# evolbioinfo/pastml

Measured on AMD Instinct MI355X. Metric: ACR nodes*states*chars/sec (full marginal pass: P(t) + bottom-up + top-down + posteriors), higher is better.
Workload: dtype f64; 1 GPU; BASELINE config 4 shard: balanced tree, 1048576 tips (2097151 nodes), k=64 states, F81, 32 characters per GPU (32 in total), marginal (BU+TD+posteriors); tips=1048576, nodes=2097151, states=64, chars_per_gpu=32, chars_total=32, substitution_model=F81, collective=local

## Files before the change

### pastml_amd/csrc/pml_api.hip

```cpp
#define PML_PLAIN_KERNELS
#include "pml_launch.h"
#include "pml_kernels_counts.h"
#include "pml_kernels_eigen_gemm.h"
#include "pml_comm.h"
#include "pml_pij_window.h"

#ifndef PML_BUILD_DIGEST
#define PML_BUILD_DIGEST "unknown"
#endif
static const char kBuildDigest[] = "PML_BUILD_DIGEST=" PML_BUILD_DIGEST;

static thread_local std::string g_last_error;

int pml_fail(int code, const char* fmt, ...) {
    char buf[1024];
    va_list ap;
    va_start(ap, fmt);
    vsnprintf(buf, sizeof(buf), fmt, ap);
    va_end(ap);
    g_last_error = buf;
    return code;
}

template <typename T>
// ... 986 lines not shown
    t.C = ctx->C;
    t.sched_cols = ctx->sched_cols;
    t.n_roots = ctx->n_roots;
    t.n_cherries = ctx->n_cherries;
    t.has_init = ctx->has_init;
    t.fuse = ctx->fuse;
    t.Gf = ctx->cols.Gf;
    t.Gt = ctx->cols.Gt;
    t.bu_wide_lanes = ctx->cols.bu_wide_lanes;
    t.level_lists_sorted = ctx->cols.level_lists_sorted;
    t.single_launch = single_launch_sweeps(ctx);
    t.blocks = block_schedule(ctx);
    t.super = super_sweeps(ctx);
    t.thin = thin_bottom_up(ctx);
    t.deep = deep_top_down(ctx);
    t.narrow_units = (int)ctx->tune.get(T_NARROW_UNITS, 0);
    t.no_td_tail = ctx->tune.on(T_NO_TD_TAIL);
    t.no_eigg_tiers = ctx->tune.on(T_NO_EIGG_TIERS);
    t.no_spin_wait = ctx->tune.on(T_NO_SPIN_WAIT);
    t.waves = PML_WAVES_PER_BLOCK;
    const int ks4 = (ctx->k + 3) / 4;
    t.eig_nb = ks4 % 4 == 0 ? 1 : (ks4 % 2 == 0 ? 2 : 4);
    t.td_chain = t.f81 && t.super && ctx->sup.chain_depth >= 0 && !ctx->tune.on(T_NO_TD_CHAIN) && !ctx->tune.on(T_NO_TD_SUPER_PIPE);
    return t;
}

static PmlSchedules schedules_of(const pml_ctx* ctx) {
    return {&ctx->blocks, &ctx->thin, &ctx->deep, &ctx->sup, &ctx->eig_tiers, &ctx->bt_tiers, &ctx->bu_level_vec_f,
            &ctx->bu_level_vec, &ctx->td_cherry_prefix};
}

static int run_plan(pml_ctx* ctx, const std::vector<PmlLaunch>& whole_plan, bool bottom_up, int is_marginal, bool force_prep) {
    const bool windowed = ctx->pij_window > 0 && ctx->kind == PML_MODEL_EIGEN;
    const int wtab = bottom_up ? 0 : 1;
    const std::vector<PmlWindowStep>* cached = nullptr;
    std::vector<PmlLaunch> cut;
    if (windowed) {
        auto same = [](const PmlLaunch& a, const PmlLaunch& b) {
            return a.op == b.op && a.list == b.list && a.kind == b.kind && a.bracket == b.bracket && a.branch == b.branch &&
                   a.signal == b.signal && a.cherries == b.cherries && a.first == b.first && a.count == b.count && a.arg == b.arg;
        };
        for (const pml_ctx::WindowCut& c : ctx->win_cuts)
            if (c.plan.size() == whole_plan.size() && std::equal(c.plan.begin(), c.plan.end(), whole_plan.begin(), same)) cached = &c.steps;
        if (cached == nullptr) {
            PmlWindowPlan W;
            const std::string bad = pml_plan_pij_window(whole_plan, ctx->forest, ctx->bu_order, ctx->td_parents, ctx->pij_window, W);
// ... 3 lines not shown
            if (ctx->win_cuts.size() >= 16) ctx->win_cuts.clear();
            ctx->win_cuts.push_back(pml_ctx::WindowCut{whole_plan, std::move(W.steps)});
            cached = &ctx->win_cuts.back().steps;
        }
        cut.reserve(cached->size());
        for (const PmlWindowStep& w : *cached) cut.push_back(w.launch);
    }
    static const std::vector<PmlWindowStep> no_steps;
    const std::vector<PmlWindowStep>& steps = windowed ? *cached : no_steps;
    const std::vector<PmlLaunch>& plan = windowed ? cut : whole_plan;
    size_t at = 0;
    const pml_ctx::EigenTiers& E = ctx->eig_tiers;
    const pml_ctx::BacktraceTiers& B = ctx->bt_tiers;
    const int* order = bottom_up ? ctx->d_bu_order : nullptr;
    const int* offsets = bottom_up ? ctx->d_bu_offsets : ctx->d_td_offsets;
    const int gemm_mode = bottom_up ? PML_EIGG_BU : PML_EIGG_TD;
    const int eig_mode = !bottom_up ? PML_EIG_TD : (is_marginal ? PML_EIG_BU_MARG : PML_EIG_BU_JOINT);
    int open = PML_NO_BRACKET;
    long long launches = 0;
    for (const PmlLaunch& r : plan) {
        if (ctx->tune.on(T_DEBUG))
            fprintf(stderr, "pml plan: branch %d op %d list %d kind %d first %d count %d arg %d bracket %d signal %d%s\n", r.branch,
                    r.op, r.list, r.kind, r.first, r.count, r.arg, r.bracket, (int)r.signal,
                    r.op == OP_SUPER && !bottom_up && r.arg > 0 ? " (chained: with the stacked units of depth arg - 1)" : "");
        if (r.bracket != open) {
            if (open != PML_NO_BRACKET) PML_TRY(prof_end(ctx, open, launches));
            if (r.bracket != PML_NO_BRACKET) PML_TRY(prof_begin(ctx));
            open = r.bracket;
            launches = 0;
        }
        ++launches;
        const PmlWindowStep* run = windowed ? &steps[at] : nullptr;
        ++at;
        if (run != nullptr && run->build_count > 0) {
            PML_TRY(launch_pij_wide_list(ctx, ctx->d_pij_window, ctx->pij_window, ctx->d_win_branches[wtab] + run->build_first,
                                         run->build_count));
            ++launches;
        }
        const bool joint = r.kind == EIG_JOINT, gemm = r.kind == EIG_GEMM;
        switch (r.op) {
            case OP_RESET_ERR:
                hipLaunchKernelGGL(reset_err_kernel, dim3((ctx->C + 63) / 64), dim3(64), 0, ctx->stream, ctx->d_err, ctx->C,
                                   r.arg ? ctx->d_tip_rest_count : nullptr);
                HIP_TRY(hipGetLastError());
                break;
            case OP_PREP:
                if (!windowed) PML_TRY(run_prep(ctx, force_prep, true));
// ... 3 lines not shown
                                   tree_of(ctx), cols_of(ctx, true), state_of(ctx), ctx->C, is_marginal ? 1 : 0, ctx->h_loglik,
                                   ctx->h_err);
                HIP_TRY(hipGetLastError());
                break;
            case OP_LEVEL:
                PML_TRY(dispatch_sweep(ctx, (SweepKind)r.kind, r.list, r.first, r.count, r.cherries, bottom_up,
                                       windowed && (r.list == L_BU_PLAIN || r.list == L_TD_PLAIN) ? wtab : -1));
                break;
            case OP_ROOTS:
                PML_TRY(dispatch_sweep(ctx, SW_ROOTS, L_NONE, 0, r.count));
                break;
            case OP_LEVELS: {
                const bool whole = r.list == L_BU_FUSED || r.list == L_TD_FUSED;
                const int do_prep = (bottom_up && r.arg && (ctx->results.pij_stale() || force_prep)) ? 1 : 0;
                PML_TRY(dispatch_small_f81(ctx, bottom_up, r.signal, do_prep, whole ? r.first : 0, r.count,
                                           whole ? nullptr : ctx->d_unit_lists[r.list], whole ? nullptr : ctx->d_list_offsets[r.list] + r.first,
                                           bottom_up ? 0 : r.arg));
                break;
            }
            case OP_BLOCKS:
                PML_TRY(dispatch_blocks_f81(ctx, bottom_up, r.first, r.signal));
                break;
            case OP_SUPER:
                PML_TRY(dispatch_super_f81(ctx, bottom_up, bottom_up ? -1 : r.arg - 1));
                break;
            case OP_STACK:
                PML_TRY(dispatch_stack_f81(ctx, bottom_up, r.first));
                break;
            case OP_EIG_TIPS:
                if (joint) PML_TRY(launch_eigen_joint_tips(ctx));
                else if (gemm) PML_TRY(launch_eigen_gemm(ctx, PML_EIGG_TIPS, ctx->d_tips, 0, ctx->n_tips));
                else PML_TRY(launch_eigen_tips(ctx, is_marginal ? 0 : 1));
                break;
            case OP_EIG_LEVEL: {
                const int* nodes = order ? order + r.first : nullptr;
                const int first = order ? 0 : r.first;
                if (joint) PML_TRY(launch_eigen_joint(ctx, ctx->d_bu_units + r.first, nullptr, 0, r.count));
                else if (gemm) PML_TRY(launch_eigen_gemm(ctx, gemm_mode, nodes, first, r.count));
                else PML_TRY(launch_eigen_fused(ctx, eig_mode, nodes, first, r.count, 0));
                break;
            }
            case OP_EIG_NARROW:
                if (joint) PML_TRY(launch_eigen_joint(ctx, ctx->d_bu_units, offsets, r.first, r.count));
                else if (gemm) PML_TRY(launch_eigen_gemm_narrow(ctx, gemm_mode, order, offsets, r.first, r.count));
                else PML_TRY(launch_eigen_narrow(ctx, eig_mode, order, offsets, r.first, r.count));
                break;
            case OP_EIG_TIER: {
// ... 1507 lines not shown
```

### pastml_amd/csrc/pml_kernels_f81.h

```cpp
#pragma once
#include "pml_device.h"
#include "pml_schedule.h"

typedef unsigned char pml_jt;

struct PmlTree {
    int N;
    int n_roots;
    const int* parent;
    const int* first_child;
    const int* n_children;
    const double* dist;
    const int* post_rank;
    const unsigned char* kind;
};

struct PmlCols {
    int k, ks, W;
    int no_wide_lean;
    const u64* masks;
    const u64* masks_init;
    const double* pi;
    const double* active;
};
// ... 1523 lines not shown
template <int G, int R>
__device__ __forceinline__ void bu_f81_super_issue(const LaneCtx<G, R>& L, const SuperRegs& s, SuperLoads<R>& ld) {
#pragma unroll
    for (int j = 0; j < 2; ++j) {
        const UnitRegs u = super_child<G>(s, j, L.g);
        f81_gather_issue<G, R>(L, u, ld.c[j].cl, ld.c[j].tl);
        ld.c[j].own = L.mask[(unsigned)u.n];
    }
    ld.e = L.E[s.fc + (L.g & 1)];
    ld.own = L.mask[(unsigned)s.n];
}

template <int R>
__device__ __forceinline__ void super_loads_arrived(SuperLoads<R>& ld) {
#pragma unroll
    for (int j = 0; j < 2; ++j)
        asm volatile("" : "+v"(ld.c[j].cl.e), "+v"(ld.c[j].cl.mask), "+v"(ld.c[j].tl.e), "+v"(ld.c[j].tl.s),
                          "+v"(ld.c[j].tl.mask), "+v"(ld.c[j].own));
    asm volatile("" : "+v"(ld.e), "+v"(ld.own));
}

template <int G, int R>
__device__ __forceinline__ bool bu_f81_super_unit(const LaneCtx<G, R>& L, const PmlTree& t, const PmlCols& c,
                                                  const PmlState& st, const SuperRegs& s, SuperLoads<R>& ld) {
    super_loads_arrived<R>(ld);
    const u64 kbits = state_bits(c.k);
    bool ones = c.k == G * R;
#pragma unroll
    for (int j = 0; j < 2; ++j) {
        f81_gather_finish<G, R>(L, ld.c[j].cl, ld.c[j].tl);
        ones = ones && (ld.c[j].own & kbits) == kbits && ld.c[j].cl.mask == kbits;
    }
    const bool full = __all(ones);
    BuResult<R> res[2];
#pragma unroll
    for (int j = 0; j < 2; ++j) {
        const UnitRegs u = super_child<G>(s, j, L.g);
        const bool ok = full ? bu_f81_marg_body<G, R, false, true, true>(L, t, c, st, u, ld.c[j], &res[j], false)
                             : bu_f81_marg_body<G, R, false, false, true>(L, t, c, st, u, ld.c[j], &res[j], false);
        if (!ok) return false;
    }
    BuLoads<R> top;
    top.cl.e = ld.e;
    top.cl.s = (L.g & 1) ? res[1].s : res[0].s;
    top.cl.be = (L.g & 1) ? res[1].e : res[0].e;
    top.cl.mask = kbits;
    top.tl.e = top.tl.s = top.tl.a = 0.0;
    top.tl.mask = 0ull;
    top.own = ld.own;
#pragma unroll
    for (int r = 0; r < R; ++r) {
        top.v0[r] = res[0].v[r];
        top.v1[r] = res[1].v[r];
    }
    return bu_f81_marg_body<G, R, true, false>(L, t, c, st, super_own(s), top);
}

template <int G, int R>
__device__ __forceinline__ void bu_f81_super_seq(const LaneCtx<G, R>& L, const PmlTree& t, const PmlCols& c,
                                                 const PmlState& st, const SuperRegs& s) {
    bu_f81_unit_seq<G, R, false>(L, t, c, st, super_child<G>(s, 0, L.g));
    bu_f81_unit_seq<G, R, false>(L, t, c, st, super_child<G>(s, 1, L.g));
    __threadfence();
    bu_f81_unit_seq<G, R, false>(L, t, c, st, super_own(s));
}

template <int G, int R>
__global__ void __launch_bounds__(PML_BLOCK) __attribute__((amdgpu_waves_per_eu(2, 2)))
bu_f81_super_kernel(PmlTree t, PmlCols c, PmlState st, const PmlUnit* __restrict__ units, int n_level) {
    constexpr int UW = 64 / G;
    const int wave = threadIdx.x >> 6;
    const int sub = (threadIdx.x & 63) / G;
    LaneCtx<G, R> L;
    lane_ctx_init<G, R>(L, t, c, st);
    const int stride = gridDim.x * PML_WAVES_PER_BLOCK * UW;
    int idx = (blockIdx.x * PML_WAVES_PER_BLOCK + wave) * UW + sub;
    int base = idx - sub;
    SuperRegs ua = load_super(units, idx < n_level ? idx : 0);
// ... 950 lines not shown
    int n, fc, g0, g1;
};

__device__ __forceinline__ StackRegs load_stack(const PmlUnit* __restrict__ units, int idx) {
    const int4 h = *reinterpret_cast<const int4*>(units + idx);
    const int4 f = *reinterpret_cast<const int4*>(units[idx].cfc);
    StackRegs s;
    s.n = h.x;
    s.fc = h.y;
    s.g0 = f.x;
    s.g1 = f.y;
    return s;
}

__device__ __forceinline__ UnitRegs stack_child(const StackRegs& s, int j) {
    UnitRegs u;
    u.n = s.fc + j;
    u.fc = j ? s.g1 : s.g0;
    u.packed = PML_PACKED_TWO_STORED;
    u.cfc = u.cfc1 = u.cfc2 = u.cfc3 = 0;
    return u;
}

template <int G, int R>
__device__ __forceinline__ void stack_child_loads(const LaneCtx<G, R>& L, const PmlCols& c, int node, int first,
                                                  BuLoads<R>& ld) {
    const int ch = first + (L.g & 1);
    ld.cl.e = L.E[ch];
    ld.cl.s = L.S[ch];
    ld.cl.be = L.be[ch];
    ld.cl.mask = 0ull;
    ld.tl.e = ld.tl.s = ld.tl.a = 0.0;
    ld.tl.mask = 0ull;
    ld.own = L.mask[(unsigned)node];
    node_load_vec<G, R>(L, c, L.bu, first, ld.v0);
    node_load_vec<G, R>(L, c, L.bu, first + 1, ld.v1);
}

template <int G, int R>
__device__ __forceinline__ bool bu_f81_stack_unit(const LaneCtx<G, R>& L, const PmlTree& t, const PmlCols& c,
                                                  const PmlState& st, const StackRegs& s) {
    BuLoads<R> ld[2];
#pragma unroll
    for (int j = 0; j < 2; ++j) stack_child_loads<G, R>(L, c, s.fc + j, j ? s.g1 : s.g0, ld[j]);
    const double e_top = L.E[s.fc + (L.g & 1)];
    const u64 own = L.mask[(unsigned)s.n];
    BuResult<R> res[2];
#pragma unroll
    for (int j = 0; j < 2; ++j)
        if (!bu_f81_marg_body<G, R, true, false>(L, t, c, st, stack_child(s, j), ld[j], &res[j], false)) return false;
    BuLoads<R> top;
    top.cl.e = e_top;
    top.cl.s = (L.g & 1) ? res[1].s : res[0].s;
    top.cl.be = (L.g & 1) ? res[1].e : res[0].e;
    top.cl.mask = 0ull;
    top.tl.e = top.tl.s = top.tl.a = 0.0;
    top.tl.mask = 0ull;
    top.own = own;
#pragma unroll
    for (int r = 0; r < R; ++r) {
        top.v0[r] = res[0].v[r];
        top.v1[r] = res[1].v[r];
    }
    UnitRegs un;
    un.n = s.n;
    un.fc = s.fc;
    un.packed = PML_PACKED_TWO_STORED;
    un.cfc = un.cfc1 = un.cfc2 = un.cfc3 = 0;
    return bu_f81_marg_body<G, R, true, false>(L, t, c, st, un, top);
}

template <int G, int R>
__global__ void __launch_bounds__(PML_BLOCK) __attribute__((amdgpu_waves_per_eu(2, 2)))
bu_f81_stack_kernel(PmlTree t, PmlCols c, PmlState st, const PmlUnit* __restrict__ units, int n_level) {
    constexpr int UW = 64 / G;
    const int wave = threadIdx.x >> 6;
    const int sub = (threadIdx.x & 63) / G;
    LaneCtx<G, R> L;
    lane_ctx_init<G, R>(L, t, c, st);
    const int stride = gridDim.x * PML_WAVES_PER_BLOCK * UW;
    int idx = (blockIdx.x * PML_WAVES_PER_BLOCK + wave) * UW + sub;
    StackRegs cur = load_stack(units, idx < n_level ? idx : 0);
    for (int base = idx - sub; base < n_level; base += stride) {
        const int nxt_idx = idx + stride;
        const StackRegs nxt = load_stack(units, nxt_idx < n_level ? nxt_idx : 0);
        if (idx < n_level) {
            if (!bu_f81_stack_unit<G, R>(L, t, c, st, cur)) {
                bu_f81_unit_seq<G, R, false>(L, t, c, st, stack_child(cur, 0));
                bu_f81_unit_seq<G, R, false>(L, t, c, st, stack_child(cur, 1));
                __threadfence();
                UnitRegs un = stack_child(cur, 0);
                un.n = cur.n;
                un.fc = cur.fc;
                bu_f81_unit_seq<G, R, false>(L, t, c, st, un);
            }
        }
        cur = nxt;
        idx = nxt_idx;
    }
}

struct TdRowNowhere {
    template <int G, int R>
    __device__ __forceinline__ void operator()(const LaneCtx<G, R>&, const PmlCols&, int, const double (&)[R], double, i64) const {}
};
#define PML_TD_CHAIN_SLOT(G, R) ((G) * (R) + 2)
struct TdRowToLds {
    double* slots;
    template <int G, int R>
    __device__ __forceinline__ void operator()(const LaneCtx<G, R>& L, const PmlCols& c, int jx, const double (&po)[R], double ls,
                                               i64 le) const {
        double* row = slots + jx * PML_TD_CHAIN_SLOT(G, R);
#pragma unroll
        for (int r = 0; r < R; r += 2) {
            double2 t2;
            t2.x = L.st(r) < c.ks ? po[r] : 0.0;
            t2.y = L.st(r) < c.ks ? po[r + 1] : 0.0;
            *reinterpret_cast<double2*>(row + L.st(r)) = t2;
        }
        if (L.g == 0) {
            row[G * R] = ls;
// ... 400 lines not shown
```

### pastml_amd/csrc/pml_launch.h

```cpp
#pragma once
#include "pml_host.h"
#include "pml_time_segments.h"

#define PML_GR_CASES(X)  \
    X(8, 4)              \
    X(1, 1)              \
    X(2, 1)              \
    X(4, 1)              \
    X(8, 1)              \
    X(16, 1)             \
    X(64, 1)             \
    X(32, 2)             \
    X(64, 2)             \
    X(64, 4)


#define PML_F81_CASES(X) \
    X(2, 2)              \
    X(4, 2)              \
    X(1, 1)              \
    X(1, 2)              \
    X(1, 4)              \
    X(2, 4)              \
    X(4, 4)              \
// ... 33 lines not shown

static bool eigen_gemm(const pml_ctx* c) {
    const bool off = c->tune.on(T_NO_EIGEN_GEMM) || c->tune.on(T_NO_MFMA) || c->tune.on(T_NO_EIGEN_FUSED);
    if (off || !c->eig_fused_opt || c->kind != PML_MODEL_EIGEN || c->k < 2) return false;
    if (c->k <= 64) return c->W == 1;
    return c->k <= 128 && c->W == 2 && c->eig_sym_all && c->d_Asym != nullptr;
}


static bool eigen_joint_valu(const pml_ctx* c) {
    const bool off = c->tune.on(T_NO_EIGEN_JOINT_VALU);
    return !off && c->eigj_valu_opt && c->kind == PML_MODEL_EIGEN && c->k >= 2 && c->k <= 64 && c->W == 1 &&
           c->d_AinvT != nullptr;
}


PML_INTERNAL int dispatch_sweep_matrix(pml_ctx* ctx, SweepKind what, const int* level, int n_level, int window = -1);
PML_INTERNAL int dispatch_select(pml_ctx* ctx, int method, int force_joint, const u64* d_lh_mask);
PML_INTERNAL int dispatch_sweep_f81(pml_ctx* ctx, SweepKind what, const PmlUnit* units, int n_level, bool cherries, bool bu_sweep);
PML_INTERNAL int dispatch_sweep_f81_wide(pml_ctx* ctx, SweepKind what, const PmlUnit* units, int n_level, bool cherries, bool bu_sweep);
PML_INTERNAL int dispatch_small_f81(pml_ctx* ctx, bool bottom_up, bool signal, int do_prep, int first_level, int n_levels,
                                    const PmlUnit* units = nullptr, const int* d_offsets = nullptr, int skip_roots = 0);
PML_INTERNAL int dispatch_blocks_f81(pml_ctx* ctx, bool bottom_up, int which, bool signal);
PML_INTERNAL int dispatch_super_f81(pml_ctx* ctx, bool bottom_up, int chain_depth = -1);
PML_INTERNAL int dispatch_stack_f81(pml_ctx* ctx, bool bottom_up, int level);
PML_INTERNAL int launch_eigen_fused(pml_ctx* ctx, int mode, const int* nodes, int first, int n, int tips);
PML_INTERNAL int launch_eigen_narrow(pml_ctx* ctx, int mode, const int* nodes, const int* d_offsets, int first_level, int n_levels);
PML_INTERNAL int launch_eigen_tips(pml_ctx* ctx, int joint);
PML_INTERNAL int launch_pij_mfma(pml_ctx* ctx);
PML_INTERNAL int launch_pij_wide(pml_ctx* ctx);
PML_INTERNAL int launch_pij_wide_list(pml_ctx* ctx, double* window, long long B, const int* d_branches, int count, int col_begin = 0,
                                      int col_end = -1);
PML_INTERNAL int arm_pij_wide_list(pml_ctx* ctx);
PML_INTERNAL int launch_eigen_gemm(pml_ctx* ctx, int mode, const int* nodes, int first, int n);
PML_INTERNAL int launch_eigen_gemm_narrow(pml_ctx* ctx, int mode, const int* nodes, const int* d_offsets, int first_level,
                                          int n_levels, const int* d_blk_start = nullptr, int n_blocks = 1);
PML_INTERNAL int launch_eigen_gemm_wide(pml_ctx* ctx, int mode, const int* nodes, int first, int n);
PML_INTERNAL int launch_eigen_gemm_narrow_wide(pml_ctx* ctx, int mode, const int* nodes, const int* d_offsets, int first_level,
                                               int n_levels, const int* d_blk_start, int n_blocks);
PML_INTERNAL int launch_eigen_joint(pml_ctx* ctx, const PmlUnit* units, const int* d_offsets, int first, int n,
                                    const int* d_blk_start = nullptr, int n_blocks = 1);
PML_INTERNAL int launch_eigen_joint_tips(pml_ctx* ctx);
PML_INTERNAL int launch_pij_valu(pml_ctx* ctx);
PML_INTERNAL int launch_simulate(pml_ctx* ctx, int col, int rep_offset, u64 seed, void* d_states, size_t rs);
PML_INTERNAL int sim_frontier_depth(const pml_ctx* ctx, int n_tiles);
PML_INTERNAL int sim_subtree_lists(pml_ctx* ctx, int D);
static inline bool pij_windowed(const pml_ctx* ctx) {
// ... 94 lines not shown
```

### pastml_amd/csrc/pml_launch_f81_super.hip

```cpp
#include "pml_launch.h"

template <int G, int R, bool LANES, bool PIPE>
static void launch_td_super_f81(pml_ctx* ctx, dim3 grid, const PmlTree& t, const PmlCols& c, const PmlState& st) {
    hipLaunchKernelGGL((td_f81_super_kernel<G, R, LANES, PIPE>), grid, dim3(PML_BLOCK), 0, ctx->stream, t, c, st, ctx->sup.d_units,
                       ctx->sup.n);
}

template <int G, int R>
static void launch_td_chain_f81(pml_ctx* ctx, int a, const PmlTree& t, const PmlCols& c, const PmlState& st) {
    const int tiles = (2 * ctx->sup.n + 4 * (64 / G) - 1) / (4 * (64 / G));
    dim3 grid(grid_for(ctx, tiles, PML_WAVES_PER_BLOCK, ctx->C, true), ctx->C);
    if (!ctx->tune.on(T_NO_TIP_LANES))
        hipLaunchKernelGGL((td_f81_chain_kernel<G, R, true>), grid, dim3(PML_BLOCK), 0, ctx->stream, t, c, st, ctx->sup.d_units,
                           ctx->sup.n, ctx->sup.d_stack_td + a);
    else
        hipLaunchKernelGGL((td_f81_chain_kernel<G, R, false>), grid, dim3(PML_BLOCK), 0, ctx->stream, t, c, st, ctx->sup.d_units,
                           ctx->sup.n, ctx->sup.d_stack_td + a);
}

template <int G, int R>
static void launch_super_f81(pml_ctx* ctx, bool bottom_up, int chain_first) {
    const PmlTree t = tree_of(ctx, true);
    const PmlCols c = cols_of(ctx, bottom_up);
    const PmlState st = state_of(ctx);
    if (chain_first >= 0) return launch_td_chain_f81<G, R>(ctx, chain_first, t, c, st);
    const int upb = PML_WAVES_PER_BLOCK * (64 / G);
    const bool pipe = bottom_up || !ctx->tune.on(T_NO_TD_SUPER_PIPE);
    dim3 grid(grid_for(ctx, bottom_up ? ctx->sup.n : 2 * ctx->sup.n, upb, ctx->C, pipe), ctx->C), block(PML_BLOCK);
    const bool lanes = !ctx->tune.on(T_NO_TIP_LANES);
    if (bottom_up)
        hipLaunchKernelGGL((bu_f81_super_kernel<G, R>), grid, block, 0, ctx->stream, t, c, st, ctx->sup.d_units, ctx->sup.n);
    else if (pipe && lanes)
        launch_td_super_f81<G, R, true, true>(ctx, grid, t, c, st);
    else if (pipe)
        launch_td_super_f81<G, R, false, true>(ctx, grid, t, c, st);
    else if (lanes)
        launch_td_super_f81<G, R, true, false>(ctx, grid, t, c, st);
    else
        launch_td_super_f81<G, R, false, false>(ctx, grid, t, c, st);
}

template <int G, int R>
static void launch_stack_f81(pml_ctx* ctx, bool bottom_up, int a, int n) {
    const PmlTree t = tree_of(ctx, true);
    const PmlCols c = cols_of(ctx, bottom_up);
    const PmlState st = state_of(ctx);
    const int upb = PML_WAVES_PER_BLOCK * (64 / G);
    dim3 grid(grid_for(ctx, bottom_up ? n : 2 * n, upb, ctx->C), ctx->C), block(PML_BLOCK);
    if (bottom_up)
        hipLaunchKernelGGL((bu_f81_stack_kernel<G, R>), grid, block, 0, ctx->stream, t, c, st, ctx->sup.d_stack_bu + a, n);
    else
        hipLaunchKernelGGL((td_f81_stack_kernel<G, R>), grid, block, 0, ctx->stream, t, c, st, ctx->sup.d_stack_td + a, n);
}

int dispatch_super_f81(pml_ctx* ctx, bool bottom_up, int chain_depth) {
    if (ctx->sup.n <= 0) return PML_OK;
    int chain_first = -1;
    if (chain_depth >= 0) {
        const std::vector<int>& off = ctx->sup.stack_td_offsets;
        if (bottom_up || chain_depth != ctx->sup.chain_depth || chain_depth + 1 >= (int)off.size() ||
            (long long)(off[chain_depth + 1] - off[chain_depth]) * 4 != ctx->sup.n)
            return fail(PML_ERR_INVALID, "no chained two-level launch for depth %d", chain_depth);
        chain_first = off[chain_depth];
    }
    const auto [g, r] = ctx->cols.shape(bottom_up);
#define X(G_, R_)                                                \
    if (g == G_ && r == R_) {                                    \
        launch_super_f81<G_, R_>(ctx, bottom_up, chain_first);   \
        HIP_TRY(hipGetLastError());                              \
        return PML_OK;                                           \
    }
    PML_SUPER_CASES(X)
#undef X
    return fail(PML_ERR_UNSUPPORTED, "no two-level F81 kernel for G=%d R=%d", g, r);
}

int dispatch_stack_f81(pml_ctx* ctx, bool bottom_up, int level) {
    const std::vector<int>& off = bottom_up ? ctx->sup.stack_bu_offsets : ctx->sup.stack_td_offsets;
    if (ctx->sup.n_stack == 0 || level + 1 >= (int)off.size()) return PML_OK;
    const int a = off[level], n = off[level + 1] - a;
    if (n <= 0) return PML_OK;
    const auto [g, r] = ctx->cols.shape(bottom_up);
#define X(G_, R_)                                         \
    if (g == G_ && r == R_) {                             \
        launch_stack_f81<G_, R_>(ctx, bottom_up, a, n);   \
        HIP_TRY(hipGetLastError());                       \
// ... 8 lines not shown
```

### pastml_amd/csrc/pml_schedule.cpp

```cpp
#include "pml_schedule.h"
#include "pml_columns.h"

#include <algorithm>
#include <cstdarg>
#include <cstdio>

static std::string message(const char* fmt, ...) __attribute__((format(printf, 1, 2)));
static std::string message(const char* fmt, ...) {
    char buf[1024];
    va_list ap;
    va_start(ap, fmt);
    vsnprintf(buf, sizeof(buf), fmt, ap);
    va_end(ap);
    return buf;
}

std::string pml_check_tree(const PmlTreeArrays& t) {
    const int n_nodes = t.n_nodes, n_roots = t.n_roots, n_bu_levels = t.n_bu_levels, n_td_levels = t.n_td_levels;
    const int *parent = t.parent, *first_child = t.first_child, *n_children = t.n_children, *bu_offsets = t.bu_offsets,
              *bu_order = t.bu_order, *td_offsets = t.td_offsets, *td_parent_offsets = t.td_parent_offsets,
              *td_parents = t.td_parents, *post_rank = t.post_rank;
    if (n_nodes <= 0 || n_roots <= 0 || n_roots > n_nodes) return "bad node/root counts";
    if (!parent || !first_child || !n_children || !t.dist || !bu_offsets || !td_offsets || !td_parent_offsets || !post_rank)
        return "NULL tree array";
// ... 453 lines not shown
        const std::vector<int> depth_of = node_depths(f);
        U.stack_bu_offsets.assign(max_h + 1, 0);
        for (int n : stack_list) ++U.stack_bu_offsets[fh[n]];
        for (int l = 0; l < max_h; ++l) U.stack_bu_offsets[l + 1] += U.stack_bu_offsets[l];
        std::vector<int> by_depth(stack_list);
        std::stable_sort(by_depth.begin(), by_depth.end(), [&](int x, int y) { return depth_of[x] < depth_of[y]; });
        U.stack_td_offsets.assign(n_td_levels + 1, 0);
        for (int n : by_depth) ++U.stack_td_offsets[depth_of[n] + 1];
        for (int l = 0; l < n_td_levels; ++l) U.stack_td_offsets[l + 1] += U.stack_td_offsets[l];
        P.sup.stack_bu = describe(f, stack_list);
        P.sup.stack_td = describe(f, by_depth);
        P.sup.stack_children = describe(f, stack_children);
        U.n_stack = (int)stack_list.size();
        int deepest = n_td_levels - 1;
        while (deepest >= 0 && U.stack_td_offsets[deepest + 1] == U.stack_td_offsets[deepest]) --deepest;
        const int a = U.stack_td_offsets[deepest], cnt = U.stack_td_offsets[deepest + 1] - a;
        bool lined_up = (long long)cnt * 4 == (long long)sup_list.size();
        for (int m = 0; m < cnt && lined_up; ++m) {
            const int n = by_depth[a + m], g0 = fc[fc[n]], g1 = fc[fc[n] + 1];
            lined_up = sup_list[4 * m] == g0 && sup_list[4 * m + 1] == g0 + 1 && sup_list[4 * m + 2] == g1 &&
                       sup_list[4 * m + 3] == g1 + 1;
        }
        if (lined_up) U.chain_depth = deepest;
        if (tune.on(T_DEBUG)) fprintf(stderr, "pastml_hip: %d stacked units, chain depth %d\n", U.n_stack, U.chain_depth);
    }
    if (sup_list.empty() && stack_list.empty()) return;
    std::vector<int> bu_r, td_r;
    U.bu_offsets_r.assign(1, 0);
    for (int l = 0; l < max_h; ++l) {
        for (int q = off[l]; q < off[l + 1]; ++q)
            if (!gone[order[q]]) bu_r.push_back(order[q]);
        U.bu_offsets_r.push_back((int)bu_r.size());
    }
    U.td_offsets_r.assign(1, 0);
    for (int l = 0; l < n_td_levels; ++l) {
        for (int q = f.td_parent_offsets_f[l]; q < f.td_parent_offsets_f[l + 1]; ++q)
            if (!gone[f.tdp[q]]) td_r.push_back(f.tdp[q]);
        U.td_offsets_r.push_back((int)td_r.size());
    }
    for (int n : sup_list) {
        sup_children.push_back(fc[n]);
        sup_children.push_back(fc[n] + 1);
    }
    U.n_child_units = (int)sup_children.size();
    P.sup.child_units = describe(f, sup_children);
    P.sup.bu_units_r = describe(f, bu_r);
    P.sup.td_units_r = describe(f, td_r);
// ... 313 lines not shown
    };
    auto narrow_end = [&](int list, int first_level, int tail) {
        p.bracket = PML_NO_BRACKET;
        if (tail > 0) p.add(OP_LEVELS, list, first_level, tail).signal = t.sched_cols <= 64 && !t.no_spin_wait;
    };
    switch (p.branch) {
        case BU_ONE_LAUNCH: {
            PmlLaunch& r = p.add(OP_LEVELS, L_BU_FUSED, 0, nl);
            r.arg = 1;
            r.signal = t.sched_cols <= 64 && !t.no_spin_wait;
            break;
        }
        case BU_BLOCKS: {
            const PmlBlockSchedule& B = *s.blocks;
            p.add(OP_BLOCKS, L_NONE, 0, B.n_blocks);
            const int n = (int)B.top_bu_offsets.size() - 1;
            const int tail = narrow_levels(t, B.top_bu_offsets, n, false, t.sched_cols);
            p.levels(OP_LEVEL, L_TOP_BU, B.top_bu_offsets, 0, n - tail, true, marg_kind(B.top_bu_vec));
            narrow_end(L_TOP_BU, n - tail, tail);
            break;
        }
        case BU_SUPER: {
            const PmlSuperSchedule& U = *s.sup;
            p.bracket = 4;
            if (U.n > 0) p.add(OP_SUPER, L_NONE, 0, U.n);
            p.bracket = 0;
            const int n = (int)U.bu_offsets_r.size() - 1;
            int tail = narrow_levels(t, U.bu_offsets_r, n, false, t.sched_cols);
            for (int l = n - 1; l >= 0 && U.n_stack > 0; --l)
                if (U.stack_bu_offsets[l + 1] > U.stack_bu_offsets[l]) {
                    tail = std::min(tail, n - 1 - l);
                    break;
                }
            if (tail < 2) tail = 0;
            p.levels(OP_LEVEL, t.level_lists_sorted ? L_REST_BU_SORTED : L_REST_BU, U.bu_offsets_r, 0, n - tail, false,
                     marg_kind(U.bu_level_vec_r), [&](int l) { add_stack(p, U, U.stack_bu_offsets, l); });
            narrow_end(L_REST_BU, n - tail, tail);
            break;
        }
        case BU_THIN: {
            const PmlThinSchedule& H = *s.thin;
            p.levels(OP_LEVEL, fused_list, f.bu_offsets_f, 0, H.floor_level, true, marg_kind(*s.bu_level_vec_f));
            for (size_t q = 0; q < H.tiers.size(); ++q) p.add(OP_BLOCKS, L_NONE, 1 + (int)q, H.tiers[q].n_blocks);
            const int tail = std::min(nl - H.top_level, narrow_levels(t, f.bu_offsets_f, nl, false, t.sched_cols));
            p.levels(OP_LEVEL, fused_list, f.bu_offsets_f, H.top_level, nl - tail, true, marg_kind(*s.bu_level_vec_f));
            narrow_end(L_BU_FUSED, nl - tail, tail);
            break;
        }
        case BU_FUSED: {
            const int tail = narrow_levels(t, f.bu_offsets_f, nl, false, t.sched_cols);
            p.levels(OP_LEVEL, fused_list, f.bu_offsets_f, 0, nl - tail, true, marg_kind(*s.bu_level_vec_f));
            narrow_end(L_BU_FUSED, nl - tail, tail);
            break;
        }
        case BU_FUSED_JOINT:
            p.levels(OP_LEVEL, L_BU_FUSED, f.bu_offsets_f, 0, nl, true,
                     [&](int l) { return (int)((*s.bu_level_vec_f)[l] ? SW_BU_JOINT_FUSED : SW_BU_JOINT_FUSED_NOVEC); });
            break;
        case BU_EIGJ_TIERS:
// ... 129 lines not shown
```

### pastml_amd/csrc/pml_schedule.h

```cpp
#pragma once
#include <cstdlib>
#include <string>
#include <vector>

#define PML_KIND_TIP 0
#define PML_KIND_CHERRY 1
#define PML_KIND_STORED 2

struct __attribute__((aligned(32))) PmlUnit {
    int n, fc, packed, pad;
    int cfc[4];
};

#define PML_PACKED_TWO_STORED ((1 << 11) | (1 << 8) | (3 << 4) | 2)

#define PML_SMALL_BLOCK 512

#define PML_TUNABLES(X)                                                                                              \
    X(GRID_CAP, 0, 0) X(SMALL_MANY_NODES, 0, 0) X(BLOCK_MAX_WORK, 0, 0)    \
    X(NO_MFMA, 1, 0) X(NO_EIGEN_FUSED, 1, 0) X(NO_HKY_FUSED, 1, 0)      \
    X(BLOCK_THREADS, 0, 0) X(EIG_BLOCKS, 0, 0) X(NO_EIGEN_GEMM, 1, 0) X(NO_EIGEN_JOINT_VALU, 1, 0) X(EIGJ_BLOCKS, 0, 0) \
    X(EIGJ_TIP_BLOCKS, 0, 0) X(EIGJ_ONE_TIPS_KERNEL, 1, 0) X(EIGJ_TIER_THIN, 0, 1) X(EIGJ_TIER_DEPTH, 0, 1)            \
    X(NO_EIGJ_TIERS, 1, 1) X(NO_BT_TIERS, 1, 1) X(NO_SHAPE_SORT, 1, 1) X(NO_SUPER, 1, 1) X(SUPER_MIN, 0, 1)            \
    X(STACK_MIN, 0, 1) X(NO_STACK, 1, 1) X(DEBUG, 1, 0) X(BLOCK_NODES, 0, 1) X(BLOCK_MAX_STORED, 0, 1)                 \
    X(BLOCK_HEIGHT_CAP, 0, 1) X(SMALL_MAX_NODES, 0, 1) X(F81_R, 0, 1) X(F81_TD_R, 0, 1) X(NO_GRAPH, 1, 1)              \
    X(NARROW_UNITS, 0, 0) X(NO_EIGG_TIERS, 1, 0) X(NO_SPIN_WAIT, 1, 0)   \
    X(PIJ_STAGE_ROWS, 0, 0) X(PIJ_BLOCKS, 0, 0) X(NO_HEIGHT_ORDER, 1, 1) X(NO_TD_TAIL, 1, 0) X(NO_PIJ_VALU, 1, 0) X(PIJ_VALU, 1, 0) X(NO_PIJ_WIDE, 1, 0) X(NO_EIGJ_PIPE, 1, 0) \
    X(THIN_UNITS, 0, 1) X(THIN_BYTES, 0, 1) X(THIN_BLOCK_NODES, 0, 1) X(NO_THIN, 1, 0) X(NO_THIN_WIDE, 1, 0) X(BU_WIDE, 0, 1) X(SORT_LEVELS, 0, 1) X(NO_WIDE_LEAN, 1, 0) X(SHAPE_ORDER, 0, 1) \
    X(PARS_MAX_COLS, 0, 0) X(PARS_THIN, 0, 0) X(COMPRESS_MAX_COLS, 0, 0) X(COMPRESS_PLAIN_ATOMICS, 1, 0) \
    X(PIJ_WINDOW, 0, 0) X(NO_KEEP_TIP_ROWS, 1, 0) X(NO_TIP_LANES, 1, 0) X(NO_TD_SUPER_PIPE, 1, 0) X(NO_TD_CHAIN, 1, 0)
enum PmlTunable {
#define X(name, flag, tree) T_##name,
    PML_TUNABLES(X)
#undef X
    T_COUNT
};
static const char* const kTunableName[T_COUNT] = {
#define X(name, flag, tree) #name,
    PML_TUNABLES(X)
#undef X
};
static const bool kTunableFlag[T_COUNT] = {
#define X(name, flag, tree) flag != 0,
    PML_TUNABLES(X)
#undef X
};
static const bool kTunableTree[T_COUNT] = {
#define X(name, flag, tree) tree != 0,
    PML_TUNABLES(X)
#undef X
};
struct PmlTune {
    long long val[T_COUNT];
// ... 29 lines not shown
    struct Tier { int first_block, n_blocks; };
    std::vector<Tier> tiers;
    PmlUnit* d_units = nullptr;
    int *d_start = nullptr, *d_levels = nullptr, *d_lv = nullptr;
};
struct PmlDeepSchedule {
    bool ok = false;
    int first_depth = 0, n_blocks = 0;
    PmlUnit* d_units = nullptr;
    int *d_start = nullptr, *d_levels = nullptr, *d_lv = nullptr;
};
struct PmlSuperSchedule {
    bool ok = false;
    int n = 0;
    PmlUnit* d_units = nullptr;
    PmlUnit* d_child_units = nullptr;
    PmlUnit *d_bu_units_r = nullptr, *d_td_units_r = nullptr;
    PmlUnit *d_bu_units_rs = nullptr, *d_td_units_rs = nullptr;
    int n_child_units = 0;
    int n_stack = 0;
    PmlUnit *d_stack_bu = nullptr, *d_stack_td = nullptr, *d_stack_children = nullptr;
    std::vector<int> stack_bu_offsets, stack_td_offsets;
    int chain_depth = -1;
    int *d_bu_offsets_r = nullptr, *d_td_offsets_r = nullptr;
    std::vector<int> bu_offsets_r, td_offsets_r;
    std::vector<char> bu_level_vec_r;
};
struct PmlEigenTiers {
    bool ok = false;
    int first_level = 0;
    int top_level = 0;
    struct Tier { int first_block, n_blocks, depth; };
    std::vector<Tier> tiers;
    PmlUnit* d_units = nullptr;
    int *d_lv = nullptr, *d_start = nullptr;
    int* d_nodes = nullptr;
    int widest = 0;
};
struct PmlBacktraceTiers {
    bool ok = false;
    int first_depth = 0;
    struct Tier { int first_block, n_blocks, depth; };
    std::vector<Tier> tiers;
    int *d_nodes = nullptr, *d_lv = nullptr, *d_start = nullptr;
};

// ... 126 lines not shown
struct PmlSweepOutcome {
    int n_signals = 0;
    bool final_signals = false;
    bool has_params = false;
    bool fused_joint = false;
    void then(const PmlSweepOutcome& next) {
        n_signals += next.n_signals;
        final_signals = next.final_signals;
        has_params = has_params || next.has_params;
        fused_joint = fused_joint || next.fused_joint;
    }
};
struct PmlSweepTraits {
    bool f81, eigen_fused, eigen_gemm, eigen_joint_valu, hky_fused, wide_states;
    int k, W, C, sched_cols, n_roots, n_cherries;
    bool has_init, fuse;
    int Gf, Gt;
    bool bu_wide_lanes, level_lists_sorted;
    bool single_launch, blocks, super, thin, deep;
    int narrow_units;
    bool no_td_tail, no_eigg_tiers, no_spin_wait;
    int waves, eig_nb;
    bool td_chain;
};
struct PmlSchedules {
    const PmlBlockSchedule* blocks;
    const PmlThinSchedule* thin;
    const PmlDeepSchedule* deep;
    const PmlSuperSchedule* sup;
    const PmlEigenTiers* eig;
    const PmlBacktraceTiers* bt;
    const std::vector<char>*bu_level_vec_f, *bu_level_vec;
    const std::vector<int>* td_cherry_prefix;
};

#define PML_PLAN __attribute__((visibility("hidden")))
PML_PLAN std::string pml_check_tree(const PmlTreeArrays& t);
PML_PLAN PmlForest pml_plan_forest(PmlTreeArrays& t, const PmlTune& tune, bool fuse, PmlNumbering& num);
PML_PLAN PmlTreePlan pml_plan_tree(const PmlForest& f, const PmlTreeArrays& t, const PmlTune& tune);
PML_PLAN PmlThinPlan pml_plan_thin_ends(const PmlForest& f, const PmlTune& tune, int thin);
PML_PLAN std::vector<PmlLaunch> pml_plan_bottom_up(const PmlForest& f, const PmlSchedules& s, const PmlSweepTraits& t, bool is_marginal);
PML_PLAN std::vector<PmlLaunch> pml_plan_top_down(const PmlForest& f, const PmlSchedules& s, const PmlSweepTraits& t, bool wants_signal);
PML_PLAN std::vector<PmlLaunch> pml_plan_backtrace(const PmlForest& f, const PmlSchedules& s, const PmlSweepTraits& t, int* head);
PML_PLAN PmlSweepOutcome pml_plan_outcome(const std::vector<PmlLaunch>& plan);
```

Measured before the change: 628.8 billion node*state*char/s.

## Chain bottom-up super units with the first stacked level via LDS in one kernel

Adds a bottom-up chained kernel that processes four super units per stacked unit and passes their partial likelihood vectors and scale scalars through shared memory to the stacked parent, instead of writing them to global memory and launching a separate stack kernel. The scheduler detects when the lowest stacked level lines up exactly with the super list and skips that level's separate stack launch. Loads for the stack step (edge factors, masks) are prefetched while the supers run. This removes a kernel launch and a global round trip of child vectors, but it adds LDS use, fixes 2 waves per block and needs a fallback path from global memory when any lane had to take the sequential route.

```diff
diff --git a/pastml_amd/csrc/pml_api.hip b/pastml_amd/csrc/pml_api.hip
--- a/pastml_amd/csrc/pml_api.hip
+++ b/pastml_amd/csrc/pml_api.hip
@@ -1032,6 +1032,7 @@
     const int ks4 = (ctx->k + 3) / 4;
     t.eig_nb = ks4 % 4 == 0 ? 1 : (ks4 % 2 == 0 ? 2 : 4);
     t.td_chain = t.f81 && t.super && ctx->sup.chain_depth >= 0 && !ctx->tune.on(T_NO_TD_CHAIN) && !ctx->tune.on(T_NO_TD_SUPER_PIPE);
+    t.bu_chain = t.f81 && t.super && ctx->sup.bu_chain_level >= 0 && !ctx->tune.on(T_NO_BU_CHAIN);
     return t;
 }
 
@@ -1081,7 +1082,8 @@
         if (ctx->tune.on(T_DEBUG))
             fprintf(stderr, "pml plan: branch %d op %d list %d kind %d first %d count %d arg %d bracket %d signal %d%s\n", r.branch,
                     r.op, r.list, r.kind, r.first, r.count, r.arg, r.bracket, (int)r.signal,
-                    r.op == OP_SUPER && !bottom_up && r.arg > 0 ? " (chained: with the stacked units of depth arg - 1)" : "");
+                    r.op != OP_SUPER || r.arg <= 0 ? "" : bottom_up ? " (chained: with the stacked units of level arg - 1)"
+                                                                    : " (chained: with the stacked units of depth arg - 1)");
         if (r.bracket != open) {
             if (open != PML_NO_BRACKET) PML_TRY(prof_end(ctx, open, launches));
             if (r.bracket != PML_NO_BRACKET) PML_TRY(prof_begin(ctx));
@@ -1131,7 +1133,7 @@
                 PML_TRY(dispatch_blocks_f81(ctx, bottom_up, r.first, r.signal));
                 break;
             case OP_SUPER:
-                PML_TRY(dispatch_super_f81(ctx, bottom_up, bottom_up ? -1 : r.arg - 1));
+                PML_TRY(dispatch_super_f81(ctx, bottom_up, r.arg - 1));
                 break;
             case OP_STACK:
                 PML_TRY(dispatch_stack_f81(ctx, bottom_up, r.first));
diff --git a/pastml_amd/csrc/pml_kernels_f81.h b/pastml_amd/csrc/pml_kernels_f81.h
--- a/pastml_amd/csrc/pml_kernels_f81.h
+++ b/pastml_amd/csrc/pml_kernels_f81.h
@@ -1569,7 +1569,8 @@
 
 template <int G, int R>
 __device__ __forceinline__ bool bu_f81_super_unit(const LaneCtx<G, R>& L, const PmlTree& t, const PmlCols& c,
-                                                  const PmlState& st, const SuperRegs& s, SuperLoads<R>& ld) {
+                                                  const PmlState& st, const SuperRegs& s, SuperLoads<R>& ld,
+                                                  BuResult<R>* keep = nullptr) {
     super_loads_arrived<R>(ld);
     const u64 kbits = state_bits(c.k);
     bool ones = c.k == G * R;
@@ -1600,7 +1601,7 @@
         top.v0[r] = res[0].v[r];
         top.v1[r] = res[1].v[r];
     }
-    return bu_f81_marg_body<G, R, true, false>(L, t, c, st, super_own(s), top);
+    return bu_f81_marg_body<G, R, true, false>(L, t, c, st, super_own(s), top, keep, true);
 }
 
 template <int G, int R>
@@ -2597,29 +2598,111 @@
     return u;
 }
 
-template <int G, int R>
+struct BuKidsFromMemory {
+    template <int G, int R>
+    __device__ __forceinline__ void scalars(const LaneCtx<G, R>& L, int, int ch, double& s, i64& be) const {
+        s = L.S[ch];
+        be = L.be[ch];
+    }
+    template <int G, int R>
+    __device__ __forceinline__ void vectors(const LaneCtx<G, R>& L, const PmlCols& c, int, int first, double (&v0)[R],
+                                            double (&v1)[R]) const {
+        node_load_vec<G, R>(L, c, L.bu, first, v0);
+        node_load_vec<G, R>(L, c, L.bu, first + 1, v1);
+    }
+};
+#define PML_BU_CHAIN_SLOT(G, R) ((G) * (R) + 2)
+struct BuKidsFromLds {
+    const double* slots;
+    template <int G, int R>
+    __device__ __forceinline__ void scalars(const LaneCtx<G, R>& L, int j, int, double& s, i64& be) const {
+        const double* row = slots + (2 * j + (L.g & 1)) * PML_BU_CHAIN_SLOT(G, R);
+        s = row[G * R];
+        be = *reinterpret_cast<const i64*>(row + G * R + 1);
+    }
+    template <int G, int R>
+    __device__ __forceinline__ void vectors(const LaneCtx<G, R>& L, const PmlCols&, int j, int, double (&v0)[R],
+                                            double (&v1)[R]) const {
+        const double* row = slots + 2 * j * PML_BU_CHAIN_SLOT(G, R);
+#pragma unroll
+        for (int r = 0; r < R; r += 2) {
+            const double2 a = *reinterpret_cast<const double2*>(row + L.st(r));
+            const double2 b = *reinterpret_cast<const double2*>(row + PML_BU_CHAIN_SLOT(G, R) + L.st(r));
+            v0[r] = a.x;
+            v0[r + 1] = a.y;
+            v1[r] = b.x;
+            v1[r + 1] = b.y;
+        }
+    }
+};
+struct BuKidsOfChain {
+    const double* slots;
+    bool from_memory;
+    template <int G, int R>
+    __device__ __forceinline__ void scalars(const LaneCtx<G, R>& L, int j, int ch, double& s, i64& be) const {
+        if (from_memory) BuKidsFromMemory().scalars<G, R>(L, j, ch, s, be);
+        else BuKidsFromLds{slots}.scalars<G, R>(L, j, ch, s, be);
+    }
+    template <int G, int R>
+    __device__ __forceinline__ void vectors(const LaneCtx<G, R>& L, const PmlCols& c, int j, int first, double (&v0)[R],
+                                            double (&v1)[R]) const {
+        if (from_memory) BuKidsFromMemory().vectors<G, R>(L, c, j, first, v0, v1);
+        else BuKidsFromLds{slots}.vectors<G, R>(L, c, j, first, v0, v1);
+    }
+};
+template <int G, int R>
+__device__ __forceinline__ void bu_chain_slot_store(const LaneCtx<G, R>& L, const PmlCols& c, double* row, const BuResult<R>& res) {
+#pragma unroll
+    for (int r = 0; r < R; r += 2) {
+        double2 t2;
+        t2.x = L.st(r) < c.ks ? res.v[r] : 0.0;
+        t2.y = L.st(r) < c.ks ? res.v[r + 1] : 0.0;
+        *reinterpret_cast<double2*>(row + L.st(r)) = t2;
+    }
+    if (L.g == 0) {
+        row[G * R] = res.s;
+        *reinterpret_cast<i64*>(row + G * R + 1) = res.e;
+    }
+}
+
+struct StackAhead {
+    double e[2], e_top;
+    u64 own[2], own_top;
+};
+template <int G, int R>
+__device__ __forceinline__ void stack_ahead_issue(const LaneCtx<G, R>& L, const StackRegs& s, StackAhead& a) {
+#pragma unroll
+    for (int j = 0; j < 2; ++j) {
+        a.e[j] = L.E[(j ? s.g1 : s.g0) + (L.g & 1)];
+        a.own[j] = L.mask[(unsigned)(s.fc + j)];
+    }
+    a.e_top = L.E[s.fc + (L.g & 1)];
+    a.own_top = L.mask[(unsigned)s.n];
+}
+
+template <int G, int R, class Kids = BuKidsFromMemory>
 __device__ __forceinline__ void stack_child_loads(const LaneCtx<G, R>& L, const PmlCols& c, int node, int first,
-                                                  BuLoads<R>& ld) {
+                                                  BuLoads<R>& ld, const Kids& kids = Kids(), int j = 0,
+                                                  const StackAhead* ahead = nullptr) {
     const int ch = first + (L.g & 1);
-    ld.cl.e = L.E[ch];
-    ld.cl.s = L.S[ch];
-    ld.cl.be = L.be[ch];
+    ld.cl.e = ahead != nullptr ? ahead->e[j] : L.E[ch];
+    kids.template scalars<G, R>(L, j, ch, ld.cl.s, ld.cl.be);
     ld.cl.mask = 0ull;
     ld.tl.e = ld.tl.s = ld.tl.a = 0.0;
     ld.tl.mask = 0ull;
-    ld.own = L.mask[(unsigned)node];
-    node_load_vec<G, R>(L, c, L.bu, first, ld.v0);
-    node_load_vec<G, R>(L, c, L.bu, first + 1, ld.v1);
-}
-
-template <int G, int R>
+    ld.own = ahead != nullptr ? ahead->own[j] : L.mask[(unsigned)node];
+    kids.template vectors<G, R>(L, c, j, first, ld.v0, ld.v1);
+}
+
+template <int G, int R, class Kids = BuKidsFromMemory>
 __device__ __forceinline__ bool bu_f81_stack_unit(const LaneCtx<G, R>& L, const PmlTree& t, const PmlCols& c,
-                                                  const PmlState& st, const StackRegs& s) {
+                                                  const PmlState& st, const StackRegs& s, const Kids& kids = Kids(),
+                                                  const StackAhead* ahead = nullptr) {
     BuLoads<R> ld[2];
 #pragma unroll
-    for (int j = 0; j < 2; ++j) stack_child_loads<G, R>(L, c, s.fc + j, j ? s.g1 : s.g0, ld[j]);
-    const double e_top = L.E[s.fc + (L.g & 1)];
-    const u64 own = L.mask[(unsigned)s.n];
+    for (int j = 0; j < 2; ++j) stack_child_loads<G, R>(L, c, s.fc + j, j ? s.g1 : s.g0, ld[j], kids, j, ahead);
+    const double e_top = ahead != nullptr ? ahead->e_top : L.E[s.fc + (L.g & 1)];
+    const u64 own = ahead != nullptr ? ahead->own_top : L.mask[(unsigned)s.n];
     BuResult<R> res[2];
 #pragma unroll
     for (int j = 0; j < 2; ++j)
@@ -2643,6 +2726,18 @@
     un.packed = PML_PACKED_TWO_STORED;
     un.cfc = un.cfc1 = un.cfc2 = un.cfc3 = 0;
     return bu_f81_marg_body<G, R, true, false>(L, t, c, st, un, top);
+}
+
+template <int G, int R>
+__device__ __forceinline__ void bu_f81_stack_seq(const LaneCtx<G, R>& L, const PmlTree& t, const PmlCols& c,
+                                                 const PmlState& st, const StackRegs& s) {
+    bu_f81_unit_seq<G, R, false>(L, t, c, st, stack_child(s, 0));
+    bu_f81_unit_seq<G, R, false>(L, t, c, st, stack_child(s, 1));
+    __threadfence();
+    UnitRegs un = stack_child(s, 0);
+    un.n = s.n;
+    un.fc = s.fc;
+    bu_f81_unit_seq<G, R, false>(L, t, c, st, un);
 }
 
 template <int G, int R>
@@ -2660,18 +2755,86 @@
         const int nxt_idx = idx + stride;
         const StackRegs nxt = load_stack(units, nxt_idx < n_level ? nxt_idx : 0);
         if (idx < n_level) {
-            if (!bu_f81_stack_unit<G, R>(L, t, c, st, cur)) {
-                bu_f81_unit_seq<G, R, false>(L, t, c, st, stack_child(cur, 0));
-                bu_f81_unit_seq<G, R, false>(L, t, c, st, stack_child(cur, 1));
-                __threadfence();
-                UnitRegs un = stack_child(cur, 0);
-                un.n = cur.n;
-                un.fc = cur.fc;
-                bu_f81_unit_seq<G, R, false>(L, t, c, st, un);
-            }
+            if (!bu_f81_stack_unit<G, R>(L, t, c, st, cur)) bu_f81_stack_seq<G, R>(L, t, c, st, cur);
         }
         cur = nxt;
         idx = nxt_idx;
+    }
+}
+
+#define PML_BU_CHAIN_WAVES 2
+template <int G, int R>
+__global__ void __launch_bounds__(64 * PML_BU_CHAIN_WAVES) __attribute__((amdgpu_waves_per_eu(2, 2)))
+bu_f81_chain_kernel(PmlTree t, PmlCols c, PmlState st, const PmlUnit* __restrict__ units, int n_level,
+                    const PmlUnit* __restrict__ stack_units) {
+    constexpr int UW = 64 / G, SLOT = PML_BU_CHAIN_SLOT(G, R);
+    const int wave = threadIdx.x >> 6;
+    const int sub = (threadIdx.x & 63) / G;
+    __shared__ __attribute__((aligned(16))) double node_vecs[PML_BU_CHAIN_WAVES * 4 * UW * SLOT];
+    double* const wave_vecs = node_vecs + wave * (4 * UW * SLOT);
+    LaneCtx<G, R> L;
+    lane_ctx_init<G, R>(L, t, c, st);
+    const int n_stack = n_level / 4;
+    const int n_tiles = (n_stack + UW - 1) / UW;
+    const int stride = gridDim.x * PML_BU_CHAIN_WAVES;
+    auto super_desc = [&](int q, int p) {
+        const int i = (4 * q + p) * UW + sub;
+        return load_super(units, i < n_level ? i : 0);
+    };
+    auto pass = [&](int q, int p, const SuperRegs& s, SuperLoads<R>& ld) {
+        if ((4 * q + p) * UW + sub >= n_level) return false;
+        BuResult<R> res;
+        if (bu_f81_super_unit<G, R>(L, t, c, st, s, ld, &res)) {
+            bu_chain_slot_store<G, R>(L, c, wave_vecs + (p * UW + sub) * SLOT, res);
+            return false;
+        }
+        bu_f81_super_seq<G, R>(L, t, c, st, s);
+        return true;
+    };
+    int q = blockIdx.x * PML_BU_CHAIN_WAVES + wave;
+    SuperRegs ua = super_desc(q, 0), ub = super_desc(q, 1);
+    SuperLoads<R> la, lb;
+    bu_f81_super_issue<G, R>(L, ua, la);
+    for (; q < n_tiles; q += stride) {
+        bool seq = false;
+        const StackRegs sk = load_stack(stack_units, q * UW + sub < n_stack ? q * UW + sub : 0);
+        {
+            const SuperRegs un = super_desc(q, 2);
+            bu_f81_super_issue<G, R>(L, ub, lb);
+            seq |= pass(q, 0, ua, la);
+            ua = un;
+        }
+        {
+            const SuperRegs un = super_desc(q, 3);
+            bu_f81_super_issue<G, R>(L, ua, la);
+            seq |= pass(q, 1, ub, lb);
+            ub = un;
+        }
+        {
+            const SuperRegs un = super_desc(q + stride, 0);
+            bu_f81_super_issue<G, R>(L, ub, lb);
+            seq |= pass(q, 2, ua, la);
+            ua = un;
+        }
+        const int m = q * UW + sub;
+        {
+            const SuperRegs un = super_desc(q + stride, 1);
+            bu_f81_super_issue<G, R>(L, ua, la);
+            seq |= pass(q, 3, ub, lb);
+            ub = un;
+        }
+        StackAhead ahead;
+        stack_ahead_issue<G, R>(L, sk, ahead);
+        wave_sync_lds();
+        const bool from_memory = __any(seq);
+        if (from_memory) __threadfence();
+        if (m < n_stack) {
+            if (!bu_f81_stack_unit<G, R>(L, t, c, st, sk, BuKidsOfChain{wave_vecs + 4 * sub * SLOT, from_memory}, &ahead)) {
+                if (!from_memory) __threadfence();
+                bu_f81_stack_seq<G, R>(L, t, c, st, sk);
+            }
+        }
+        wave_sync_lds();
     }
 }
 
diff --git a/pastml_amd/csrc/pml_launch.h b/pastml_amd/csrc/pml_launch.h
--- a/pastml_amd/csrc/pml_launch.h
+++ b/pastml_amd/csrc/pml_launch.h
@@ -79,7 +79,7 @@
 PML_INTERNAL int dispatch_small_f81(pml_ctx* ctx, bool bottom_up, bool signal, int do_prep, int first_level, int n_levels,
                                     const PmlUnit* units = nullptr, const int* d_offsets = nullptr, int skip_roots = 0);
 PML_INTERNAL int dispatch_blocks_f81(pml_ctx* ctx, bool bottom_up, int which, bool signal);
-PML_INTERNAL int dispatch_super_f81(pml_ctx* ctx, bool bottom_up, int chain_depth = -1);
+PML_INTERNAL int dispatch_super_f81(pml_ctx* ctx, bool bottom_up, int chain = -1);
 PML_INTERNAL int dispatch_stack_f81(pml_ctx* ctx, bool bottom_up, int level);
 PML_INTERNAL int launch_eigen_fused(pml_ctx* ctx, int mode, const int* nodes, int first, int n, int tips);
 PML_INTERNAL int launch_eigen_narrow(pml_ctx* ctx, int mode, const int* nodes, const int* d_offsets, int first_level, int n_levels);
diff --git a/pastml_amd/csrc/pml_launch_f81_super.hip b/pastml_amd/csrc/pml_launch_f81_super.hip
--- a/pastml_amd/csrc/pml_launch_f81_super.hip
+++ b/pastml_amd/csrc/pml_launch_f81_super.hip
@@ -19,10 +19,19 @@
 }
 
 template <int G, int R>
+static void launch_bu_chain_f81(pml_ctx* ctx, int a, const PmlTree& t, const PmlCols& c, const PmlState& st) {
+    const int tiles = (ctx->sup.n + 4 * (64 / G) - 1) / (4 * (64 / G));
+    dim3 grid(grid_for(ctx, tiles, PML_BU_CHAIN_WAVES, ctx->C, true), ctx->C);
+    hipLaunchKernelGGL((bu_f81_chain_kernel<G, R>), grid, dim3(64 * PML_BU_CHAIN_WAVES), 0, ctx->stream, t, c, st, ctx->sup.d_units,
+                       ctx->sup.n, ctx->sup.d_stack_bu + a);
+}
+
+template <int G, int R>
 static void launch_super_f81(pml_ctx* ctx, bool bottom_up, int chain_first) {
     const PmlTree t = tree_of(ctx, true);
     const PmlCols c = cols_of(ctx, bottom_up);
     const PmlState st = state_of(ctx);
+    if (chain_first >= 0 && bottom_up) return launch_bu_chain_f81<G, R>(ctx, chain_first, t, c, st);
     if (chain_first >= 0) return launch_td_chain_f81<G, R>(ctx, chain_first, t, c, st);
     const int upb = PML_WAVES_PER_BLOCK * (64 / G);
     const bool pipe = bottom_up || !ctx->tune.on(T_NO_TD_SUPER_PIPE);
@@ -53,15 +62,15 @@
         hipLaunchKernelGGL((td_f81_stack_kernel<G, R>), grid, block, 0, ctx->stream, t, c, st, ctx->sup.d_stack_td + a, n);
 }
 
-int dispatch_super_f81(pml_ctx* ctx, bool bottom_up, int chain_depth) {
+int dispatch_super_f81(pml_ctx* ctx, bool bottom_up, int chain) {
     if (ctx->sup.n <= 0) return PML_OK;
     int chain_first = -1;
-    if (chain_depth >= 0) {
-        const std::vector<int>& off = ctx->sup.stack_td_offsets;
-        if (bottom_up || chain_depth != ctx->sup.chain_depth || chain_depth + 1 >= (int)off.size() ||
-            (long long)(off[chain_depth + 1] - off[chain_depth]) * 4 != ctx->sup.n)
-            return fail(PML_ERR_INVALID, "no chained two-level launch for depth %d", chain_depth);
-        chain_first = off[chain_depth];
+    if (chain >= 0) {
+        const std::vector<int>& off = bottom_up ? ctx->sup.stack_bu_offsets : ctx->sup.stack_td_offsets;
+        if (chain != (bottom_up ? ctx->sup.bu_chain_level : ctx->sup.chain_depth) || chain + 1 >= (int)off.size() ||
+            (long long)(off[chain + 1] - off[chain]) * 4 != ctx->sup.n)
+            return fail(PML_ERR_INVALID, "no chained two-level launch for %s %d", bottom_up ? "level" : "depth", chain);
+        chain_first = off[chain];
     }
     const auto [g, r] = ctx->cols.shape(bottom_up);
 #define X(G_, R_)                                                \
diff --git a/pastml_amd/csrc/pml_schedule.cpp b/pastml_amd/csrc/pml_schedule.cpp
--- a/pastml_amd/csrc/pml_schedule.cpp
+++ b/pastml_amd/csrc/pml_schedule.cpp
@@ -499,7 +499,19 @@
                        sup_list[4 * m + 3] == g1 + 1;
         }
         if (lined_up) U.chain_depth = deepest;
-        if (tune.on(T_DEBUG)) fprintf(stderr, "pastml_hip: %d stacked units, chain depth %d\n", U.n_stack, U.chain_depth);
+        int lowest = 0;
+        while (lowest < max_h && U.stack_bu_offsets[lowest + 1] == U.stack_bu_offsets[lowest]) ++lowest;
+        const int b = U.stack_bu_offsets[lowest], bcnt = U.stack_bu_offsets[lowest + 1] - b;
+        lined_up = (long long)bcnt * 4 == (long long)sup_list.size();
+        for (int m = 0; m < bcnt && lined_up; ++m) {
+            const int n = stack_list[b + m], g0 = fc[fc[n]], g1 = fc[fc[n] + 1];
+            lined_up = sup_list[4 * m] == g0 && sup_list[4 * m + 1] == g0 + 1 && sup_list[4 * m + 2] == g1 &&
+                       sup_list[4 * m + 3] == g1 + 1 && depth_of[n] == depth_of[stack_list[b]];
+        }
+        if (lined_up) U.bu_chain_level = lowest;
+        if (tune.on(T_DEBUG))
+            fprintf(stderr, "pastml_hip: %d stacked units, chain depth %d, bottom-up chain level %d\n", U.n_stack, U.chain_depth,
+                    U.bu_chain_level);
     }
     if (sup_list.empty() && stack_list.empty()) return;
     std::vector<int> bu_r, td_r;
@@ -859,8 +871,9 @@
         }
         case BU_SUPER: {
             const PmlSuperSchedule& U = *s.sup;
+            const int chained = t.bu_chain && U.n > 0 ? U.bu_chain_level : -1;
             p.bracket = 4;
-            if (U.n > 0) p.add(OP_SUPER, L_NONE, 0, U.n);
+            if (U.n > 0) p.add(OP_SUPER, L_NONE, 0, U.n).arg = chained + 1;
             p.bracket = 0;
             const int n = (int)U.bu_offsets_r.size() - 1;
             int tail = narrow_levels(t, U.bu_offsets_r, n, false, t.sched_cols);
@@ -871,7 +884,7 @@
                 }
             if (tail < 2) tail = 0;
             p.levels(OP_LEVEL, t.level_lists_sorted ? L_REST_BU_SORTED : L_REST_BU, U.bu_offsets_r, 0, n - tail, false,
-                     marg_kind(U.bu_level_vec_r), [&](int l) { add_stack(p, U, U.stack_bu_offsets, l); });
+                     marg_kind(U.bu_level_vec_r), [&](int l) { if (l != chained) add_stack(p, U, U.stack_bu_offsets, l); });
             narrow_end(L_REST_BU, n - tail, tail);
             break;
         }
diff --git a/pastml_amd/csrc/pml_schedule.h b/pastml_amd/csrc/pml_schedule.h
--- a/pastml_amd/csrc/pml_schedule.h
+++ b/pastml_amd/csrc/pml_schedule.h
@@ -28,7 +28,7 @@
     X(PIJ_STAGE_ROWS, 0, 0) X(PIJ_BLOCKS, 0, 0) X(NO_HEIGHT_ORDER, 1, 1) X(NO_TD_TAIL, 1, 0) X(NO_PIJ_VALU, 1, 0) X(PIJ_VALU, 1, 0) X(NO_PIJ_WIDE, 1, 0) X(NO_EIGJ_PIPE, 1, 0) \
     X(THIN_UNITS, 0, 1) X(THIN_BYTES, 0, 1) X(THIN_BLOCK_NODES, 0, 1) X(NO_THIN, 1, 0) X(NO_THIN_WIDE, 1, 0) X(BU_WIDE, 0, 1) X(SORT_LEVELS, 0, 1) X(NO_WIDE_LEAN, 1, 0) X(SHAPE_ORDER, 0, 1) \
     X(PARS_MAX_COLS, 0, 0) X(PARS_THIN, 0, 0) X(COMPRESS_MAX_COLS, 0, 0) X(COMPRESS_PLAIN_ATOMICS, 1, 0) \
-    X(PIJ_WINDOW, 0, 0) X(NO_KEEP_TIP_ROWS, 1, 0) X(NO_TIP_LANES, 1, 0) X(NO_TD_SUPER_PIPE, 1, 0) X(NO_TD_CHAIN, 1, 0)
+    X(PIJ_WINDOW, 0, 0) X(NO_KEEP_TIP_ROWS, 1, 0) X(NO_TIP_LANES, 1, 0) X(NO_TD_SUPER_PIPE, 1, 0) X(NO_TD_CHAIN, 1, 0) X(NO_BU_CHAIN, 1, 0)
 enum PmlTunable {
 #define X(name, flag, tree) T_##name,
     PML_TUNABLES(X)
@@ -104,6 +104,7 @@
     PmlUnit *d_stack_bu = nullptr, *d_stack_td = nullptr, *d_stack_children = nullptr;
     std::vector<int> stack_bu_offsets, stack_td_offsets;
     int chain_depth = -1;
+    int bu_chain_level = -1;
     int *d_bu_offsets_r = nullptr, *d_td_offsets_r = nullptr;
     std::vector<int> bu_offsets_r, td_offsets_r;
     std::vector<char> bu_level_vec_r;
@@ -276,6 +277,7 @@
     bool no_td_tail, no_eigg_tiers, no_spin_wait;
     int waves, eig_nb;
     bool td_chain;
+    bool bu_chain;
 };
 struct PmlSchedules {
     const PmlBlockSchedule* blocks;
```

Measured after the change: 645.7 billion node*state*char/s, median of 6. 1.03x the previous value.
